# will-rowe/groot

Measured on AMD Instinct MI355X. Metric: Mreads/s aligned, higher is better.
Workload: dtype u64

## Files before the change

groot_amd/csrc/hip/ctx.hpp:

```cpp
#pragma once

#include <hip/hip_runtime.h>

#include <algorithm>
#include <array>
#include <atomic>
#include <cstdlib>
#include <deque>
#include <map>
#include <memory>
#include <string>
#include <thread>
#include <vector>

#include "device_types.hpp"

using namespace groot;


template <class T> struct DevBuf {
    T *p = nullptr;
    size_t n = 0;
    hipError_t alloc(size_t count)
    {
        release();
        n = count;
        return hipMalloc((void **)&p, std::max<size_t>(count, 1) * sizeof(T));
    }
    hipError_t reserve(size_t count) { return count <= n && p ? hipSuccess : alloc(count); }
    void swap(DevBuf &o) { std::swap(p, o.p); std::swap(n, o.n); }
// ... 15 lines not shown
        n = count;
        return hipHostMalloc((void **)&p, std::max<size_t>(count, 1) * sizeof(T), hipHostMallocDefault);
    }
    hipError_t reserve(size_t count) { return count <= n && p ? hipSuccess : alloc(count); }
    void release()
    {
        if (p) (void)hipHostFree(p);
        p = nullptr;
        n = 0;
    }
    ~PinBuf() { release(); }
};

struct Knobs {
    bool no_outcome_table = false, no_text_table = false, no_sig = false, force_rccl = false, small_buffers = false, open_stats = false, poison = false, lean = false, no_path = false,
         shared_slow = false, serial_tail = false, assign_global = false, library_sort = false;
    uint32_t ec_slots = 0;
    uint32_t acov_slots = 0;
    uint32_t rescue_ec_rows = 0;
    uint32_t rescue_acov_log = 0;
    static Knobs read()
    {
        Knobs k;
        k.no_outcome_table = getenv("GROOT_NO_OUTCOME_TABLE") != nullptr; k.no_text_table = getenv("GROOT_NO_TEXT_TABLE") != nullptr;
        k.no_sig = getenv("GROOT_NO_SIG") != nullptr;                     k.force_rccl = getenv("GROOT_FORCE_RCCL") != nullptr;
        k.small_buffers = getenv("GROOT_TEST_SMALL_BUFFERS") != nullptr;  k.open_stats = getenv("GROOT_OPEN_STATS") != nullptr;
        k.poison = getenv("GROOT_TEST_POISON") != nullptr;
        k.lean = getenv("GROOT_LEAN") != nullptr;
        k.no_path = getenv("GROOT_NO_PATH_PASS") != nullptr;
        k.shared_slow = getenv("GROOT_TEST_SHARED_SLOW") != nullptr;
        k.serial_tail = getenv("GROOT_SERIAL_TAIL") != nullptr;
        k.assign_global = getenv("GROOT_TEST_ASSIGN_GLOBAL") != nullptr;
        k.library_sort = getenv("GROOT_LIBRARY_SORT") != nullptr;
        if (const char *e = getenv("GROOT_TEST_EC_SLOTS")) k.ec_slots = (uint32_t)std::min<unsigned long>(strtoul(e, nullptr, 10), 1ul << 30);
        if (const char *e = getenv("GROOT_TEST_ACOV_SLOTS")) k.acov_slots = (uint32_t)std::min<unsigned long>(strtoul(e, nullptr, 10), 1ul << 30);
        if (const char *e = getenv("GROOT_TEST_RESCUE_EC_ROWS")) k.rescue_ec_rows = (uint32_t)std::min<unsigned long>(strtoul(e, nullptr, 10), 1ul << 30);
        if (const char *e = getenv("GROOT_TEST_RESCUE_ACOV_LOG")) k.rescue_acov_log = (uint32_t)std::min<unsigned long>(strtoul(e, nullptr, 10), 1ul << 28);
        return k;
    }
};

namespace groot {
struct EcTable;
struct AcovTable;
}

struct EcBufs {
    uint32_t cap = 0;
// ... 307 lines not shown
    uint32_t seed_slots = 0;
    DevBuf<uint32_t> sort_key, sort_key_out, perm_in, todo_list, todo_count;
    DevBuf<uint32_t> long_list, long_count;
    uint32_t vcap = 0;
    uint32_t lsh_defer_rows = 0, lsh_cap = 0;
    DevBuf<unsigned long long> seed_shards;
    DevBuf<uint32_t> lsh_list, lsh_count;
    DevBuf<uint64_t> lsh_sketch;
    DevBuf<char> sort_tmp, in_tmp;
    DevBuf<uint32_t> order_buf;
    size_t order_cap = 0;
    uint32_t order_dirty_n = 0, order_dirty_begin = 0, order_dirty_end = 0;
    uint32_t ovf_cap = 0;
    DevBuf<uint32_t> trav_off;
    DevBuf<char> scan_tmp;
    uint32_t align_threads = 0, stk_depth = 0;
    DevBuf<uint64_t> stk_hdr, stk_mask;
    DevBuf<uint32_t> attempts, q_row, q_seen, q_of_row, q_nrows;
    uint32_t *attempts_ptr = nullptr;
    uint32_t att_cap = 0;
    bool att_external = false;
    Counters ct;
};

#define HIP_TRY(ctx, expr)                                                                             \
    do {                                                                                                \
        hipError_t e__ = (expr);                                                                        \
        if (e__ != hipSuccess) return fail(ctx, GROOT_E_DEVICE, "%s: %s", #expr, hipGetErrorString(e__)); \
    } while (0)

// ... 18 lines not shown
```

groot_amd/csrc/hip/device_types.hpp:

```cpp
#pragma once

#include <cstdint>

#include <hip/hip_runtime.h>

#include "groot_hip.h"

namespace groot {

constexpr int kBlock = 256;
constexpr uint32_t kEmpty = 0xFFFFFFFFu;

enum : uint32_t {
    kFlagShortRead = 1u,
    kFlagLongRead = 2u,
    kFlagSeedOverflow = 4u,
    kFlagTravOverflow = 8u,
    kFlagOrdOverflow = 16u,
    kFlagOvfOverflow = 32u,
    kFlagQOverflow = 64u,
};

constexpr uint32_t kIncrCap = 8;
constexpr uint32_t kIncrCapBig = 2048;
constexpr uint32_t kSeedShards = 64, kSeedShardStride = 16;
constexpr uint32_t kOvfShards = 256;

struct DeviceCounters {
    unsigned long long mapped, multimapped, alignments, seeds, revcomp_panics, short_reads;
    unsigned int n_trav;
    unsigned int max_seeds;
    unsigned int flags;
    unsigned int q_rows;
    unsigned int mask_words;
    unsigned int todo_reads;
    unsigned int seeded_reads;
    unsigned int tab_reads;
    unsigned int lean_reads;
    unsigned int path_reads;
    unsigned int lsh_reads;
    unsigned int long_reads;
    unsigned long long dbg[192];
};

template <int PW> struct alignas(16) NodeRec {
    uint32_t seq_off;
    uint32_t seq_len;
    uint32_t deg;
    uint8_t child_first[4];
    uint64_t first8;
    uint32_t edges[4];
    uint64_t mask[PW];
};
static_assert(sizeof(NodeRec<3>) == 64, "node record must be one 64-byte line");
static_assert(sizeof(NodeRec<11>) == 128, "wide node record must be 128 bytes");

// ... 291 lines not shown
```

groot_amd/csrc/hip/groot_hip.hip:

```cpp
#include <cstring>

#include <hip/hip_runtime.h>
#include <rocprim/rocprim.hpp>

#include <dlfcn.h>

#include <algorithm>
#include <cmath>
#include <cstdarg>
#include <cstdio>
#include <atomic>
#include <chrono>
#include <deque>
#include <iterator>
#include <array>
#include <map>
#include <tuple>
#include <memory>
#include <numeric>
#include <string>
#include <thread>
#include <vector>

#include "../common/cpus.hpp"
// ... 272 lines not shown
        return GROOT_OK;
    }
    auto sort = [&](void *tmp) {
        return small_blocks ? rocprim::radix_sort_pairs<OrderSortConfig>(tmp, tmp_bytes, c->sort_key.p, c->sort_key_out.p, c->perm_in.p, w->perm.p, s->n_reads,
                                                                         begin_bit, end_bit, c->stream)
                            : rocprim::radix_sort_pairs(tmp, tmp_bytes, c->sort_key.p, c->sort_key_out.p, c->perm_in.p, w->perm.p, s->n_reads, begin_bit, end_bit,
                                                        c->stream);
    };
    HIP_TRY(c, sort(nullptr));
    if (tmp_bytes > c->sort_tmp.n) {
        HIP_TRY(c, hipStreamSynchronize(c->stream));
        HIP_TRY(c, c->sort_tmp.alloc(tmp_bytes + tmp_bytes / 4));
    }
    HIP_TRY(c, sort(c->sort_tmp.p));
    return GROOT_OK;
}

static int launch_align_stage(groot_ctx *c, Slot *s, bool update_weights)
{
    WorkSet *w = &c->ws[s->set];
    AlignArgs a{};
    a.ix = c->dix;
    a.seq = s->seq();
    a.seq_off = s->off();
    a.n_reads = s->n_reads;
    a.first_read_id = s->first_read_id;
    a.seed_slots = c->seed_slots;
    a.seed_count = w->seed_count.p;
    a.seed_win = w->seed_win.p;
    a.perm = w->perm.p;
// ... 6 lines not shown
    a.mask_first = w->mask_first.p;
    a.trav_cnt = w->trav_cnt.p;
    a.ovf_trav = w->ovf_trav.p;
    a.ovf_mask = w->ovf_mask.p;
    a.ovf_cnt = w->ovf_cnt.p;
    a.ovf_cap = c->ovf_cap;
    if (c->vcap) { a.vitem = w->vitem.p; a.vcount = w->vcount.p; a.vcap = c->vcap; }
    a.stk_hdr = c->stk_hdr.p;
    a.stk_mask = c->stk_mask.p;
    uint32_t blocks = std::min<uint32_t>((s->n_reads + kBlock - 1) / kBlock, c->align_threads / kBlock);
    if (c->dfs_frac < kSparseBelow && c->dfs_frac * (double)s->n_reads < 16.0 * (double)(blocks * (kBlock / 64))) blocks = std::max(1u, blocks / 2);
    else if (error_batch(c, s) && blocks >= 4) blocks /= 2;
    if ((s->lean_used || s->path_used) && c->lean_left_frac < 0.25) {
        uint32_t want = (uint32_t)(c->lean_left_frac * 1.25 * (double)s->n_reads / 64.0 / (kBlock / 64)) + 1u;
        blocks = std::max(1u, std::min(blocks, std::max(want, c->n_cu)));
    }
    a.n_threads = blocks * kBlock;
    a.stk_depth = c->stk_depth;
    {
        const uint32_t stride = (2 + 4 * ((s->max_len + 27) / 16)) | 1u;
        a.lds_stride_dw = (size_t)kBlock * stride * 4 <= 64 * 1024 ? stride : 0;
    }
    if (c->tab_capture) {
        a.incr_cnt = c->incr_cnt.p; a.incr_win = c->incr_win.p; a.incr_cap = c->incr_cap;
        HIP_TRY(c, hipMemsetAsync(c->incr_cnt.p, 0, (size_t)s->n_reads * sizeof(uint32_t), c->tstream));
    }
    a.head_lanes = s->mixed_len ? 16u : 0u;
#ifndef GROOT_REFILL_ERR
#define GROOT_REFILL_ERR 48
#endif
#ifndef GROOT_REFILL_MIXED
// ... 28 lines not shown
        a.perm = w->perm2.p;
        a.n_perm = l.left_cnt;
        a.rest = w->perm.p;
        a.rest_lo = lean_blocks * (uint32_t)kBlock;
        if (c->profiling) HIP_TRY(c, hipEventRecord(s->ev[13], c->astream));
        if (c->tstream != c->astream) {
            HIP_TRY(c, hipEventRecord(s->ev_walk, c->astream));
            HIP_TRY(c, hipStreamWaitEvent(c->tstream, s->ev_walk, 0));
        }
    }
    launch_align(c->pw, a, dim3(blocks), c->tstream);
    HIP_TRY(c, hipGetLastError());
    return GROOT_OK;
}

static int launch_order_stage(groot_ctx *c, Slot *s, bool update_weights)
{
    WorkSet *w = &c->ws[s->set];
    const uint32_t n = s->n_reads;
    size_t tmp_bytes = 0;
    if (c->vcap) hipLaunchKernelGGL(split_fix_kernel, dim3(256), dim3(kBlock), 0, c->tstream, w->split_list.p, w->vcount.p, w->vitem.p, w->trav_cnt.p, n, s->d_ctr.p,
                                    w->trav_first.p, w->mask_first.p, c->pw, s->first_read_id);
    HIP_TRY(c, rocprim::exclusive_scan(nullptr, tmp_bytes, w->trav_cnt.p, c->trav_off.p, 0u, n, rocprim::plus<uint32_t>(), c->tstream));
    if (tmp_bytes > c->scan_tmp.n) {
        HIP_TRY(c, hipStreamSynchronize(c->tstream));
        HIP_TRY(c, c->scan_tmp.alloc(tmp_bytes + tmp_bytes / 4));
    }
    HIP_TRY(c, rocprim::exclusive_scan(c->scan_tmp.p, tmp_bytes, w->trav_cnt.p, c->trav_off.p, 0u, n, rocprim::plus<uint32_t>(), c->tstream));
    OrderTabArgs ot{};
    if (c->dix.out_tab) {
        ot.tab_idx = w->tab_idx.p; ot.out_tab = c->dix.out_tab; ot.stride_q = c->dix.out_stride_q; ot.first_read_id = s->first_read_id;
        ot.update_weights = update_weights ? 1 : 0;
        ot.attempts = c->attempts_ptr; ot.q_row = c->q_row.p;
        ot.q_tab = c->dix.w - c->k + 1; ot.n_windows = c->n_windows;
    }
    if (c->profiling) HIP_TRY(c, hipEventRecord(s->ev[9], c->tstream));
    hipLaunchKernelGGL(order_first_kernel, dim3(std::min<uint32_t>((n + kBlock - 1) / kBlock, 2048u)), dim3(kBlock), 0, c->tstream, w->trav_first.p,
                       w->mask_first.p, c->trav_off.p, w->trav_cnt.p, n, s->d_trav.p, s->d_mask.p, s->trav_cap, c->pw,
                       c->pw_view, s->d_ctr.p, ot);
    if (c->profiling) HIP_TRY(c, hipEventRecord(s->ev[10], c->tstream));
    if (c->vcap) hipLaunchKernelGGL(order_split_kernel, dim3(std::min<uint32_t>((c->vcap + kBlock - 1) / kBlock, 256u)), dim3(kBlock), 0, c->tstream, w->vitem.p, w->vcount.p, c->vcap, w->trav_cnt.p,
                                    c->trav_off.p, w->trav_first.p, w->mask_first.p, n, s->first_read_id, s->d_trav.p, s->d_mask.p, s->trav_cap, c->pw, c->pw_view, s->d_ctr.p);
    hipLaunchKernelGGL(order_ovf_kernel, dim3((c->ovf_cap + kBlock - 1) / kBlock, kOvfShards), dim3(kBlock), 0, c->tstream,
                       w->ovf_trav.p, w->ovf_mask.p, w->ovf_cnt.p, c->ovf_cap, c->trav_off.p, s->first_read_id, s->d_trav.p,
                       s->d_mask.p, s->trav_cap, c->pw, c->pw_view, s->d_ctr.p, w->vitem.p, n, w->vcount.p);
    HIP_TRY(c, hipGetLastError());
    if (int rc = counters_assign(c, s)) return rc;
    if (!c->prm.results_on_device) {
        const dim3 g((s->trav_cap + kBlock - 1) / kBlock);
        hipLaunchKernelGGL(mask_words_kernel, g, dim3(kBlock), 0, c->tstream, s->d_trav.p, s->d_ctr.p, s->trav_cap, c->graph_words.p, (uint32_t)c->h_graph_words.size(),
                           s->d_mwords.p);
        size_t tb = 0;
        HIP_TRY(c, rocprim::exclusive_scan(nullptr, tb, s->d_mwords.p, s->d_moff.p, 0u, s->trav_cap, rocprim::plus<uint32_t>(), c->tstream));
        if (tb > c->scan_tmp.n) {
            HIP_TRY(c, hipStreamSynchronize(c->tstream));
            HIP_TRY(c, c->scan_tmp.alloc(tb + tb / 4));
        }
        HIP_TRY(c, rocprim::exclusive_scan(c->scan_tmp.p, tb, s->d_mwords.p, s->d_moff.p, 0u, s->trav_cap, rocprim::plus<uint32_t>(), c->tstream));
        hipLaunchKernelGGL(mask_compact_kernel, g, dim3(kBlock), 0, c->tstream, s->d_trav.p, s->d_mask.p, c->pw_view, s->d_ctr.p, s->trav_cap,
                           c->graph_words.p, (uint32_t)c->h_graph_words.size(), s->d_moff.p, s->d_cmask.p, s->d_ckpt.p);
// ... 284 lines not shown
        if (int rc = run_batch_async(c, s, redo_weights)) return rc;
        redone = true;
        DeviceCounters again{};
        if (int rc = refetch(again)) return rc;
        if (have_first) {
            const uint32_t keep = first.flags & ~(kFlagOvfOverflow | kFlagTravOverflow | kFlagSeedOverflow | kFlagQOverflow);
            DeviceCounters merged = first;
            merged.n_trav = again.n_trav; merged.alignments = again.alignments; merged.seeds = again.seeds; merged.max_seeds = again.max_seeds;
            merged.flags = keep | again.flags;
            merged.q_rows = again.q_rows;
            merged.mask_words = again.mask_words;
            merged.todo_reads = again.todo_reads; merged.tab_reads = again.tab_reads; merged.lean_reads = again.lean_reads; merged.path_reads = again.path_reads;
            h = merged;
        } else h = again;
    }
    s->n_trav = s->n_reads ? h.n_trav : 0;
    if (int rc = counters_collect(c, s, redone)) return rc;
    groot_counts &o = s->counts;
    o.received = s->n_reads;
    o.mapped = h.mapped; o.multimapped = h.multimapped; o.alignments = h.alignments; o.seeds = h.seeds;
    o.travs = s->n_trav; o.revcomp_panics = h.revcomp_panics; o.short_reads = h.short_reads;
    o.full_sketch_reads = (s->sig_used || s->text_used) ? h.todo_reads : s->n_reads;
    o.walked_reads = h.seeded_reads;
    o.lean_reads = h.lean_reads;
    s->path_reads = s->path_used ? h.path_reads : 0;
    if (s->status == GROOT_OK) {
        char buf[256];
        if (h.flags & kFlagLongRead) { s->status = GROOT_E_NOSPACE; snprintf(buf, sizeof buf, "a read is longer than max_read_len=%u", c->prm.max_read_len); s->status_msg = buf; }
        else if (h.flags & kFlagOrdOverflow) { s->status = GROOT_E_NOSPACE; s->status_msg = "a read produced more than 65535 traversals"; }
        else if (h.flags & kFlagShortRead) {
// ... 51 lines not shown
        fprintf(stderr, "[groot work] phase %d: %llu steps, %.2f us per step (wall clock, per wave)\n", ph, h.dbg[27 + ph],
                h.dbg[27 + ph] ? (double)h.dbg[24 + ph] / 100.0 / (double)h.dbg[27 + ph] : 0.0);
    for (int hh = 0; hh < 2; hh++) {
        fprintf(stderr, "[groot work] %s (buckets of 2 iterations):", hh ? "round length" : "lane finish");
        for (int b = 0; b < 64; b++) fprintf(stderr, " %llu", h.dbg[64 + 64 * hh + b]);
        fprintf(stderr, "\n");
    }
#endif
    if (s->n_reads) c->trav_per_read = (double)s->n_trav / (double)s->n_reads;
    if (s->n_reads && !c->tab_capture) c->dfs_frac = (double)h.seeded_reads / (double)s->n_reads;
    if (s->n_reads && !c->tab_capture && (s->lean_used || s->path_used)) {
        const uint32_t first = s->path_used ? h.path_reads : h.lean_reads;
        c->lean_left_frac = (double)(h.seeded_reads - std::min(h.seeded_reads, first)) / (double)s->n_reads;
    }
    if (s->n_reads && (s->sig_used || s->text_used)) c->todo_frac = (double)h.todo_reads / (double)s->n_reads;
    if (s->n_reads) { c->lsh_frac = (double)h.lsh_reads / (double)s->n_reads; c->long_frac = (double)h.long_reads / (double)s->n_reads; }
    if (s->n_reads && !c->tab_capture && c->dix.text_tab) {
        c->text_hit_frac = s->text_used ? 1.0 - (double)h.todo_reads / (double)s->n_reads : (double)h.tab_reads / (double)s->n_reads;
        if (s->text_used) c->text_retry_gap = c->text_hit_frac >= 0.7 ? 8u : std::min(256u, c->text_retry_gap * 2u);
    }
    s->n_mask_bytes = s->n_trav ? h.mask_words : 0;
    if (!c->prm.results_on_device && s->n_trav) {
        c->bytes_per_trav = (double)s->n_mask_bytes / (double)s->n_trav;
        const uint32_t have = redone ? 0 : std::min(s->copied, s->n_trav);
        if (have < s->n_trav) {
            if (c->packed_travs) HIP_TRY(c, hipMemcpy(s->h_ctrav.p + have, s->d_ctrav.p + have, (size_t)(s->n_trav - have) * sizeof(groot_ctrav), hipMemcpyDeviceToHost));
            else HIP_TRY(c, hipMemcpy(s->h_trav.p + have, s->d_trav.p + have, (size_t)(s->n_trav - have) * sizeof(groot_trav), hipMemcpyDeviceToHost));
            HIP_TRY(c, hipMemcpy(s->h_ckpt.p, s->d_ckpt.p, ((size_t)s->n_trav / 256 + 1) * sizeof(uint32_t), hipMemcpyDeviceToHost));
        }
        const uint64_t have_w = redone ? 0 : std::min<uint64_t>(s->copied_bytes, s->n_mask_bytes);
// ... 875 lines not shown
```

groot_amd/csrc/hip/kernels_cov.hpp:

```cpp
#pragma once

#include "kernels_common.hpp"

namespace groot {

struct CovArgs {
    const groot_trav *trav;
    const uint64_t *mask;
    const uint64_t *seq_off;
    const DeviceCounters *ctr;
    const uint32_t *node_np_off;
    const uint2 *np;
    const uint32_t *graph_path_off;
    const uint32_t *path_len;
    const uint64_t *slot_base;
    unsigned long long *starts, *ends;
    uint32_t cap, pw, first_read_id;
};

constexpr uint32_t kCovSkipFlags = kFlagSeedOverflow | kFlagTravOverflow | kFlagOvfOverflow | kFlagQOverflow | kFlagLongRead | kFlagOrdOverflow;

__global__ __launch_bounds__(kBlock) void cov_count_kernel(CovArgs a)
{
    if (a.ctr->flags & kCovSkipFlags) return;
    const uint32_t n = min(a.ctr->n_trav, a.cap);
    for (uint32_t t = blockIdx.x * kBlock + threadIdx.x; t < n; t += gridDim.x * kBlock) {
        const groot_trav tr = a.trav[t];
        const uint32_t r = tr.read_id - a.first_read_id;
        const uint64_t m = (a.seq_off[r + 1] - a.seq_off[r]) - ((tr.flags & GROOT_TRAV_START_CLIP) ? 1u : 0u) - ((tr.flags & GROOT_TRAV_END_CLIP) ? 1u : 0u);
        const uint32_t g0 = a.graph_path_off[tr.graph_id];
        const uint64_t *mk = a.mask + (size_t)t * a.pw;
        const uint32_t j1 = a.node_np_off[tr.node + 1];
        for (uint32_t j = a.node_np_off[tr.node]; j < j1; j++) {
            const uint2 e = a.np[j];
            if (!((mk[e.x >> 6] >> (e.x & 63)) & 1ull)) continue;
// ... 13 lines not shown
```

groot_amd/csrc/hip/kernels_misc.hpp:

```cpp
#pragma once

#include "kernels_common.hpp"

namespace groot {

__global__ __launch_bounds__(kBlock) void lsh_heavy_kernel(SeedArgs a)
{
    __shared__ uint64_t sk_lds[(kBlock / 64) * kLshHeavyMaxS];
    __shared__ uint32_t aux_lds[(kBlock / 64) * (2 * kLshMaxBands + 16)];
    const DeviceIndex &ix = a.ix;
    const uint32_t S = ix.s, maxk = ix.max_k, LB = ix.l_max, n = ix.n_windows;
    const uint32_t sl = S < kRowSlots ? S : kRowSlots, nd = (sl + 5) / 6;
    const uint32_t lane = threadIdx.x & 63, wave = threadIdx.x >> 6;
    uint64_t *m = sk_lds + wave * kLshHeavyMaxS;
    uint32_t *blo = aux_lds + wave * (2 * kLshMaxBands + 16);
    uint32_t *bcum = blo + kLshMaxBands;
    uint32_t *sc = bcum + kLshMaxBands + 1;
    auto wave_sync = []() { __builtin_amdgcn_fence(__ATOMIC_SEQ_CST, "wavefront"); __builtin_amdgcn_wave_barrier(); };
    const uint32_t n_list = min(*a.lsh_count, a.lsh_cap);
    for (uint32_t hi = blockIdx.x * (kBlock / 64) + wave; hi < n_list; hi += gridDim.x * (kBlock / 64)) {
        const uint32_t li = hi;
        const uint32_t e0 = a.lsh_list[li];
        const uint32_t r = e0 & 0x7FFFFFFFu, high = e0 >> 31;
        const uint64_t o0 = a.seq_off[r];
// ... 314 lines not shown

__global__ __launch_bounds__(kBlock) void fold_tab_hist_kernel(uint32_t *__restrict__ hist, uint32_t *__restrict__ attempts, const uint32_t *__restrict__ q_row,
                                                               uint32_t q_tab, uint32_t n_windows, const DeviceCounters *ctr, uint32_t update_weights)
{
    const bool live = update_weights && !(ctr->flags & (kFlagSeedOverflow | kFlagQOverflow));
    const uint32_t row = live ? q_row[q_tab] : kEmpty;
    for (uint32_t w = blockIdx.x * kBlock + threadIdx.x; w < n_windows; w += gridDim.x * kBlock) {
        const uint32_t v = hist[w];
        if (!v) continue;
        hist[w] = 0;
        if (row != kEmpty) atomicAdd(&attempts[(size_t)row * n_windows + w], v);
    }
}


struct OrderTabArgs {
    const uint32_t *tab_idx;
    const uint4 *out_tab;
    uint32_t stride_q, first_read_id;
    uint32_t update_weights;
    uint32_t *attempts;
    const uint32_t *q_row;
    uint32_t q_tab, n_windows;
};
__global__ __launch_bounds__(kBlock) void order_first_kernel(const groot_trav *first, const uint64_t *mask_first, const uint32_t *off,
                                                           const uint32_t *cnt, uint32_t n, groot_trav *out, uint64_t *mask_out,
                                                           uint32_t cap, uint32_t pw_in, uint32_t pw_out, DeviceCounters *ctr, OrderTabArgs t)
{
    __shared__ unsigned long long red[4];
    unsigned long long alns = 0, mapped = 0, multimapped = 0, seeds = 0;
    const bool live = !(ctr->flags & (kFlagSeedOverflow | kFlagQOverflow));
    if (blockIdx.x == 0 && threadIdx.x == 0 && n) ctr->n_trav = off[n - 1] + cnt[n - 1];
    for (uint32_t r = blockIdx.x * kBlock + threadIdx.x; r < n; r += gridDim.x * kBlock) {
    const uint32_t tw = t.tab_idx ? t.tab_idx[r] : kEmpty;
    const uint32_t ti = tw == kEmpty ? kEmpty : tw & ((1u << kOutIdxBits) - 1u);
    const bool count_here = (t.update_weights & 1u) && !(tw & kTabCounted);
    const bool seeds_here = tw != kEmpty && (tw & kTabSeedsHere);
    uint32_t ns = 0;
    if (ti != kEmpty && live) {
        const uint32_t nt = cnt[r], i = off[r];
        const bool fits = i < cap && nt <= cap - i;
        if (!fits) atomicOr(&ctr->flags, kFlagTravOverflow);
        const uint32_t row = t.update_weights ? t.q_row[t.q_tab] : 0u;
        uint32_t n_ent = nt ? nt : 1u;
        for (uint32_t j = 0; j < n_ent; j++) {
            const uint4 *e = t.out_tab + (size_t)(ti + j) * t.stride_q;
            uint4 h = e[0];
            if (j == 0) { n_ent += h.z >> 20; h.z &= 0xFFFFFu; }
            const uint4 x = e[1];
            const uint4 y = pw_out > 1 ? e[2] : make_uint4(0, 0, 0, 0);
            if (count_here) {
                if (x.x != kEmpty) atomicAdd(&t.attempts[(size_t)row * t.n_windows + x.x], 1u);
                if (x.y != kEmpty) atomicAdd(&t.attempts[(size_t)row * t.n_windows + x.y], 1u);
            }
            if (seeds_here) ns += (h.w >> 10) & 7u;
            if (j == 0) { mapped += (h.w >> 9) & 1u; multimapped += (h.w >> 8) & 1u; }
            if (j < nt) {
                alns += __popc(x.z) + __popc(x.w) + __popc(y.x) + __popc(y.y) + __popc(y.z) + __popc(y.w);
                if (pw_out > 3) {
                    const uint32_t *ew = reinterpret_cast<const uint32_t *>(e) + kOutHdrDw;
                    for (uint32_t w = 6; w < 2 * pw_out; w++) alns += __popc(ew[w]);
                }
            }
            if (!fits || j >= nt) continue;
            groot_trav tr;
            tr.read_id = t.first_read_id + r; tr.graph_id = h.z; tr.node = h.x; tr.offset = h.y;
            tr.ord = (uint16_t)j; tr.flags = (uint8_t)h.w; tr.reserved = 0;
            uint64_t *mo = mask_out + (size_t)(i + j) * pw_out;
            static_assert(sizeof(groot_trav) == 20, "record is five dwords");
            uint32_t tw5[5];
            __builtin_memcpy(tw5, &tr, 20);
            uint32_t *po = reinterpret_cast<uint32_t *>(out + i + j);
#pragma unroll
            for (int d = 0; d < 5; d++) __builtin_nontemporal_store(tw5[d], po + d);
            __builtin_nontemporal_store((uint64_t)x.z | ((uint64_t)x.w << 32), mo);
            if (pw_out > 1) __builtin_nontemporal_store((uint64_t)y.x | ((uint64_t)y.y << 32), mo + 1);
            if (pw_out > 2) __builtin_nontemporal_store((uint64_t)y.z | ((uint64_t)y.w << 32), mo + 2);
            const uint32_t *ew = reinterpret_cast<const uint32_t *>(e) + kOutHdrDw;
            for (uint32_t w = 3; w < pw_out; w++) mo[w] = (uint64_t)ew[2 * w] | ((uint64_t)ew[2 * w + 1] << 32);
        }
        if (seeds_here) seeds += ns;
    } else if (ti == kEmpty && cnt[r] != 0) {
        const uint32_t i = off[r];
        if (i >= cap) atomicOr(&ctr->flags, kFlagTravOverflow);
        else {
            out[i] = first[r];
            for (uint32_t w = 0; w < pw_out; w++) mask_out[(size_t)i * pw_out + w] = mask_first[(size_t)r * pw_in + w];
        }
    }
    }
    if (!t.tab_idx) return;
    alns = block_sum(alns, red);
    mapped = block_sum(mapped, red);
    multimapped = block_sum(multimapped, red);
    seeds = block_sum(seeds, red);
    if (threadIdx.x == 0) {
        if (alns) atomicAdd(&ctr->alignments, alns);
        if (seeds) atomicAdd(&ctr->seeds, seeds);
        if (t.update_weights) {
            if (mapped) atomicAdd(&ctr->mapped, mapped);
            if (multimapped) atomicAdd(&ctr->multimapped, multimapped);
        }
    }
}

__global__ __launch_bounds__(kBlock) void order_ovf_kernel(const groot_trav *ovf, const uint64_t *ovf_mask, const uint32_t *ovf_cnt,
                                                         uint32_t ovf_cap, const uint32_t *off, uint32_t first_read_id, groot_trav *out,
                                                         uint64_t *mask_out, uint32_t cap, uint32_t pw_in, uint32_t pw_out,
                                                         DeviceCounters *ctr, const uint4 *vitem, uint32_t n_reads, uint32_t *vcount)
{
    const uint32_t shard = blockIdx.y;
    const uint32_t slot = blockIdx.x * kBlock + threadIdx.x;
    if (!slot && !shard) { vcount[0] = 0; vcount[1] = 0; }
    if (slot >= min(ovf_cnt[shard], ovf_cap)) return;
    const size_t o = (size_t)shard * ovf_cap + slot;
    groot_trav t = ovf[o];
    uint32_t rid = t.read_id - first_read_id, ord = t.ord;
    if (rid >= n_reads) {
        const uint4 vi = vitem[rid - n_reads];
        rid = vi.x; ord += vi.w;
        t.read_id = first_read_id + rid;
        t.ord = (uint16_t)ord;
    }
    const uint32_t i = off[rid] + ord;
    if (i >= cap) { atomicOr(&ctr->flags, kFlagTravOverflow); return; }
    out[i] = t;
    for (uint32_t w = 0; w < pw_out; w++) mask_out[(size_t)i * pw_out + w] = ovf_mask[o * pw_in + w];
}

__global__ __launch_bounds__(kBlock) void mask_words_kernel(const groot_trav *__restrict__ trav, const DeviceCounters *ctr, uint32_t cap,
                                                          const uint8_t *__restrict__ graph_words, uint32_t n_graphs, uint32_t *__restrict__ words)
{
    const uint32_t i = blockIdx.x * kBlock + threadIdx.x;
    if (i >= cap) return;
    uint32_t w = 0;
    if (i < min(ctr->n_trav, cap)) {
        const uint32_t g = trav[i].graph_id;
        w = g < n_graphs ? graph_words[g] : 0u;
    }
    words[i] = w;
}
__global__ __launch_bounds__(kBlock) void mask_compact_kernel(const groot_trav *__restrict__ trav, const uint64_t *__restrict__ mask, uint32_t pw_in,
// ... 15 lines not shown
```

groot_amd/csrc/hip/open.hip:

```cpp
#include <hip/hip_runtime.h>

#include <algorithm>
#include <chrono>
#include <cstdio>
#include <cstring>
#include <memory>
#include <numeric>
#include <string>
#include <thread>
#include <vector>

#include "../common/cpus.hpp"
#include "../common/view_check.hpp"
#include "counters.hpp"
#include "ctx.hpp"
#include "index_tables.hpp"
#include "kernels_open.hpp"
#include "kernels_path.hpp"
#include "launch.hpp"
#include "open.hpp"

using namespace groot;

static int text_pass(groot_ctx *c, const uint8_t *seqs, const uint32_t *owner, uint32_t n, uint32_t len, uint8_t *differs, uint32_t *cnt_flags,
// ... 546 lines not shown
        HIP_TRY(c, w.perm_count.alloc(4));
        if (c->lean || c->path) {
            HIP_TRY(c, w.perm2.alloc(R));
            HIP_TRY(c, w.packed.alloc((size_t)R * (c->prm.max_read_len <= 128 ? 2 : 4)));
        }
        if (c->prm.keep_sketches) HIP_TRY(c, w.sketches.alloc((size_t)R * s));
        HIP_TRY(c, w.trav_first.alloc((size_t)R + c->vcap));
        HIP_TRY(c, w.mask_first.alloc(((size_t)R + c->vcap) * c->pw));
        HIP_TRY(c, w.trav_cnt.alloc((size_t)R + c->vcap));
        HIP_TRY(c, w.vitem.alloc(std::max<uint32_t>(c->vcap, 1)));
        HIP_TRY(c, w.split_list.alloc(kLongListCap));
        HIP_TRY(c, w.vcount.alloc(4));
        HIP_TRY(c, hipMemset(w.vcount.p, 0, 4 * sizeof(uint32_t)));
    }
    HIP_TRY(c, c->trav_off.alloc(R));
    if (c->lean || c->path) HIP_TRY(c, c->lean_stk.alloc((size_t)R * 4));
    if (c->path) HIP_TRY(c, c->path_hold.alloc((size_t)R * 3 * kPathHold));
    for (WorkSet &w : c->ws) {
        HIP_TRY(c, w.ovf_cnt.alloc(kOvfShards + 3));
        HIP_TRY(c, hipMemset(w.ovf_cnt.p, 0, (kOvfShards + 3) * sizeof(uint32_t)));
    }
    if (int rc = alloc_ovf(c, c->kn.small_buffers ? 2u : std::max<uint32_t>(256, R / kOvfShards / 4))) return rc;
    int n_cu = 256;
    (void)hipDeviceGetAttribute(&n_cu, hipDeviceAttributeMultiprocessorCount, c->device);
    c->n_cu = (uint32_t)std::max(n_cu, 1);
    uint32_t per_cu = c->pw > 3 ? kAlignWavesWide : kAlignWaves;
    c->align_threads = std::min<uint32_t>(((R + kBlock - 1) / kBlock) * kBlock, (uint32_t)std::max(n_cu, 1) * per_cu * kBlock);
    c->stk_depth = c->prm.max_read_len;
    HIP_TRY(c, c->stk_hdr.alloc((size_t)c->stk_depth * c->align_threads));
    HIP_TRY(c, c->stk_mask.alloc((size_t)c->stk_depth * c->align_threads * c->pw));
// ... 299 lines not shown
```

Baseline: 2449.

## Fuse exclusive scan into order placement kernel with decoupled look-back

```diff
diff --git a/groot_amd/csrc/hip/ctx.hpp b/groot_amd/csrc/hip/ctx.hpp
--- a/groot_amd/csrc/hip/ctx.hpp
+++ b/groot_amd/csrc/hip/ctx.hpp
@@ -14,6 +14,7 @@
 #include <vector>
 
 #include "device_types.hpp"
+#include "order_place_state.hpp"
 
 using namespace groot;
 
@@ -59,7 +60,9 @@
 
 struct Knobs {
     bool no_outcome_table = false, no_text_table = false, no_sig = false, force_rccl = false, small_buffers = false, open_stats = false, poison = false, lean = false, no_path = false,
-         shared_slow = false, serial_tail = false, assign_global = false, library_sort = false;
+         shared_slow = false, serial_tail = false, assign_global = false, library_sort = false, library_scan = false;
+    int tail_wg_per_cu = -1;
+    uint32_t tail_blocks = 0;
     uint32_t ec_slots = 0;
     uint32_t acov_slots = 0;
     uint32_t rescue_ec_rows = 0;
@@ -77,6 +80,9 @@
         k.serial_tail = getenv("GROOT_SERIAL_TAIL") != nullptr;
         k.assign_global = getenv("GROOT_TEST_ASSIGN_GLOBAL") != nullptr;
         k.library_sort = getenv("GROOT_LIBRARY_SORT") != nullptr;
+        k.library_scan = getenv("GROOT_LIBRARY_SCAN") != nullptr;
+        if (const char *e = getenv("GROOT_TAIL_WG_PER_CU")) k.tail_wg_per_cu = (int)std::min<unsigned long>(strtoul(e, nullptr, 10), 64ul);
+        if (const char *e = getenv("GROOT_TEST_TAIL_BLOCKS")) k.tail_blocks = (uint32_t)std::min<unsigned long>(strtoul(e, nullptr, 10), 1ul << 16);
         if (const char *e = getenv("GROOT_TEST_EC_SLOTS")) k.ec_slots = (uint32_t)std::min<unsigned long>(strtoul(e, nullptr, 10), 1ul << 30);
         if (const char *e = getenv("GROOT_TEST_ACOV_SLOTS")) k.acov_slots = (uint32_t)std::min<unsigned long>(strtoul(e, nullptr, 10), 1ul << 30);
         if (const char *e = getenv("GROOT_TEST_RESCUE_EC_ROWS")) k.rescue_ec_rows = (uint32_t)std::min<unsigned long>(strtoul(e, nullptr, 10), 1ul << 30);
@@ -414,6 +420,8 @@
     uint32_t ovf_cap = 0;
     DevBuf<uint32_t> trav_off;
     DevBuf<char> scan_tmp;
+    groot::order_place::State place;
+    int64_t ovf_longest = -1;
     uint32_t align_threads = 0, stk_depth = 0;
     DevBuf<uint64_t> stk_hdr, stk_mask;
     DevBuf<uint32_t> attempts, q_row, q_seen, q_of_row, q_nrows;
diff --git a/groot_amd/csrc/hip/device_types.hpp b/groot_amd/csrc/hip/device_types.hpp
--- a/groot_amd/csrc/hip/device_types.hpp
+++ b/groot_amd/csrc/hip/device_types.hpp
@@ -19,6 +19,7 @@
     kFlagOrdOverflow = 16u,
     kFlagOvfOverflow = 32u,
     kFlagQOverflow = 64u,
+    kFlagScanStall = 128u,
 };
 
 constexpr uint32_t kIncrCap = 8;
@@ -40,6 +41,7 @@
     unsigned int path_reads;
     unsigned int lsh_reads;
     unsigned int long_reads;
+    unsigned int ovf_longest;
     unsigned long long dbg[192];
 };
 
diff --git a/groot_amd/csrc/hip/groot_hip.hip b/groot_amd/csrc/hip/groot_hip.hip
--- a/groot_amd/csrc/hip/groot_hip.hip
+++ b/groot_amd/csrc/hip/groot_hip.hip
@@ -310,6 +310,11 @@
     }
     HIP_TRY(c, sort(c->sort_tmp.p));
     return GROOT_OK;
+}
+
+static uint32_t tail_wg_per_cu_default(const groot_ctx *, const Slot *)
+{
+    return 0;
 }
 
 static int launch_align_stage(groot_ctx *c, Slot *s, bool update_weights)
@@ -346,7 +351,10 @@
     if ((s->lean_used || s->path_used) && c->lean_left_frac < 0.25) {
         uint32_t want = (uint32_t)(c->lean_left_frac * 1.25 * (double)s->n_reads / 64.0 / (kBlock / 64)) + 1u;
         blocks = std::max(1u, std::min(blocks, std::max(want, c->n_cu)));
-    }
+        const uint32_t per_cu = c->kn.tail_wg_per_cu >= 0 ? (uint32_t)c->kn.tail_wg_per_cu : tail_wg_per_cu_default(c, s);
+        if (per_cu) blocks = std::max(1u, std::min(blocks, per_cu * c->n_cu));
+    }
+    if (c->kn.tail_blocks) blocks = std::max(1u, std::min(blocks, c->kn.tail_blocks));
     a.n_threads = blocks * kBlock;
     a.stk_depth = c->stk_depth;
     {
@@ -405,6 +413,14 @@
     return GROOT_OK;
 }
 
+static uint32_t ovf_blocks(uint32_t ovf_cap, int64_t longest)
+{
+    const uint32_t full = std::max<uint32_t>((ovf_cap + kBlock - 1) / kBlock, 1u);
+    if (longest < 0) return full;
+    const uint64_t want = ((uint64_t)longest + (uint64_t)longest / 4 + kBlock - 1) / kBlock;
+    return (uint32_t)std::min<uint64_t>(std::max<uint64_t>(want, 1), full);
+}
+
 static int launch_order_stage(groot_ctx *c, Slot *s, bool update_weights)
 {
     WorkSet *w = &c->ws[s->set];
@@ -412,12 +428,14 @@
     size_t tmp_bytes = 0;
     if (c->vcap) hipLaunchKernelGGL(split_fix_kernel, dim3(256), dim3(kBlock), 0, c->tstream, w->split_list.p, w->vcount.p, w->vitem.p, w->trav_cnt.p, n, s->d_ctr.p,
                                     w->trav_first.p, w->mask_first.p, c->pw, s->first_read_id);
-    HIP_TRY(c, rocprim::exclusive_scan(nullptr, tmp_bytes, w->trav_cnt.p, c->trav_off.p, 0u, n, rocprim::plus<uint32_t>(), c->tstream));
-    if (tmp_bytes > c->scan_tmp.n) {
-        HIP_TRY(c, hipStreamSynchronize(c->tstream));
-        HIP_TRY(c, c->scan_tmp.alloc(tmp_bytes + tmp_bytes / 4));
-    }
-    HIP_TRY(c, rocprim::exclusive_scan(c->scan_tmp.p, tmp_bytes, w->trav_cnt.p, c->trav_off.p, 0u, n, rocprim::plus<uint32_t>(), c->tstream));
+    if (c->kn.library_scan) {
+        HIP_TRY(c, rocprim::exclusive_scan(nullptr, tmp_bytes, w->trav_cnt.p, c->trav_off.p, 0u, n, rocprim::plus<uint32_t>(), c->tstream));
+        if (tmp_bytes > c->scan_tmp.n) {
+            HIP_TRY(c, hipStreamSynchronize(c->tstream));
+            HIP_TRY(c, c->scan_tmp.alloc(tmp_bytes + tmp_bytes / 4));
+        }
+        HIP_TRY(c, rocprim::exclusive_scan(c->scan_tmp.p, tmp_bytes, w->trav_cnt.p, c->trav_off.p, 0u, n, rocprim::plus<uint32_t>(), c->tstream));
+    }
     OrderTabArgs ot{};
     if (c->dix.out_tab) {
         ot.tab_idx = w->tab_idx.p; ot.out_tab = c->dix.out_tab; ot.stride_q = c->dix.out_stride_q; ot.first_read_id = s->first_read_id;
@@ -426,15 +444,14 @@
         ot.q_tab = c->dix.w - c->k + 1; ot.n_windows = c->n_windows;
     }
     if (c->profiling) HIP_TRY(c, hipEventRecord(s->ev[9], c->tstream));
-    hipLaunchKernelGGL(order_first_kernel, dim3(std::min<uint32_t>((n + kBlock - 1) / kBlock, 2048u)), dim3(kBlock), 0, c->tstream, w->trav_first.p,
-                       w->mask_first.p, c->trav_off.p, w->trav_cnt.p, n, s->d_trav.p, s->d_mask.p, s->trav_cap, c->pw,
-                       c->pw_view, s->d_ctr.p, ot);
+    HIP_TRY(c, order_place::launch(c->kn.library_scan ? nullptr : &c->place, w->trav_first.p, w->mask_first.p, c->trav_off.p, w->trav_cnt.p, n, s->d_trav.p, s->d_mask.p,
+                                   s->trav_cap, c->pw, c->pw_view, s->d_ctr.p, ot, c->tstream));
     if (c->profiling) HIP_TRY(c, hipEventRecord(s->ev[10], c->tstream));
     if (c->vcap) hipLaunchKernelGGL(order_split_kernel, dim3(std::min<uint32_t>((c->vcap + kBlock - 1) / kBlock, 256u)), dim3(kBlock), 0, c->tstream, w->vitem.p, w->vcount.p, c->vcap, w->trav_cnt.p,
                                     c->trav_off.p, w->trav_first.p, w->mask_first.p, n, s->first_read_id, s->d_trav.p, s->d_mask.p, s->trav_cap, c->pw, c->pw_view, s->d_ctr.p);
-    hipLaunchKernelGGL(order_ovf_kernel, dim3((c->ovf_cap + kBlock - 1) / kBlock, kOvfShards), dim3(kBlock), 0, c->tstream,
+    hipLaunchKernelGGL(order_ovf_kernel, dim3(ovf_blocks(c->ovf_cap, c->ovf_longest), kOvfShards), dim3(kBlock), 0, c->tstream,
                        w->ovf_trav.p, w->ovf_mask.p, w->ovf_cnt.p, c->ovf_cap, c->trav_off.p, s->first_read_id, s->d_trav.p,
-                       s->d_mask.p, s->trav_cap, c->pw, c->pw_view, s->d_ctr.p, w->vitem.p, n, w->vcount.p);
+                       s->d_mask.p, s->trav_cap, c->pw, c->pw_view, s->d_ctr.p, w->vitem.p, n, w->vcount.p, c->place.ticket);
     HIP_TRY(c, hipGetLastError());
     if (int rc = counters_assign(c, s)) return rc;
     if (!c->prm.results_on_device) {
@@ -749,6 +766,11 @@
             h = merged;
         } else h = again;
     }
+    if (s->n_reads && (h.flags & kFlagScanStall)) {
+        s->status = GROOT_E_DEVICE;
+        s->status_msg = "the order stage's look-back did not finish: the batch's records were not placed";
+        h.n_trav = 0;
+    }
     s->n_trav = s->n_reads ? h.n_trav : 0;
     if (int rc = counters_collect(c, s, redone)) return rc;
     groot_counts &o = s->counts;
@@ -830,6 +852,7 @@
         c->lean_left_frac = (double)(h.seeded_reads - std::min(h.seeded_reads, first)) / (double)s->n_reads;
     }
     if (s->n_reads && (s->sig_used || s->text_used)) c->todo_frac = (double)h.todo_reads / (double)s->n_reads;
+    if (s->n_reads) c->ovf_longest = h.ovf_longest;
     if (s->n_reads) { c->lsh_frac = (double)h.lsh_reads / (double)s->n_reads; c->long_frac = (double)h.long_reads / (double)s->n_reads; }
     if (s->n_reads && !c->tab_capture && c->dix.text_tab) {
         c->text_hit_frac = s->text_used ? 1.0 - (double)h.todo_reads / (double)s->n_reads : (double)h.tab_reads / (double)s->n_reads;
diff --git a/groot_amd/csrc/hip/kernels_cov.hpp b/groot_amd/csrc/hip/kernels_cov.hpp
--- a/groot_amd/csrc/hip/kernels_cov.hpp
+++ b/groot_amd/csrc/hip/kernels_cov.hpp
@@ -18,7 +18,7 @@
     uint32_t cap, pw, first_read_id;
 };
 
-constexpr uint32_t kCovSkipFlags = kFlagSeedOverflow | kFlagTravOverflow | kFlagOvfOverflow | kFlagQOverflow | kFlagLongRead | kFlagOrdOverflow;
+constexpr uint32_t kCovSkipFlags = kFlagSeedOverflow | kFlagTravOverflow | kFlagOvfOverflow | kFlagQOverflow | kFlagLongRead | kFlagOrdOverflow | kFlagScanStall;
 
 __global__ __launch_bounds__(kBlock) void cov_count_kernel(CovArgs a)
 {
diff --git a/groot_amd/csrc/hip/kernels_misc.hpp b/groot_amd/csrc/hip/kernels_misc.hpp
--- a/groot_amd/csrc/hip/kernels_misc.hpp
+++ b/groot_amd/csrc/hip/kernels_misc.hpp
@@ -1,6 +1,7 @@
 #pragma once
 
 #include "kernels_common.hpp"
+#include "order_place.hpp"
 
 namespace groot {
 
@@ -352,105 +353,18 @@
 }
 
 
-struct OrderTabArgs {
-    const uint32_t *tab_idx;
-    const uint4 *out_tab;
-    uint32_t stride_q, first_read_id;
-    uint32_t update_weights;
-    uint32_t *attempts;
-    const uint32_t *q_row;
-    uint32_t q_tab, n_windows;
-};
-__global__ __launch_bounds__(kBlock) void order_first_kernel(const groot_trav *first, const uint64_t *mask_first, const uint32_t *off,
-                                                           const uint32_t *cnt, uint32_t n, groot_trav *out, uint64_t *mask_out,
-                                                           uint32_t cap, uint32_t pw_in, uint32_t pw_out, DeviceCounters *ctr, OrderTabArgs t)
-{
-    __shared__ unsigned long long red[4];
-    unsigned long long alns = 0, mapped = 0, multimapped = 0, seeds = 0;
-    const bool live = !(ctr->flags & (kFlagSeedOverflow | kFlagQOverflow));
-    if (blockIdx.x == 0 && threadIdx.x == 0 && n) ctr->n_trav = off[n - 1] + cnt[n - 1];
-    for (uint32_t r = blockIdx.x * kBlock + threadIdx.x; r < n; r += gridDim.x * kBlock) {
-    const uint32_t tw = t.tab_idx ? t.tab_idx[r] : kEmpty;
-    const uint32_t ti = tw == kEmpty ? kEmpty : tw & ((1u << kOutIdxBits) - 1u);
-    const bool count_here = (t.update_weights & 1u) && !(tw & kTabCounted);
-    const bool seeds_here = tw != kEmpty && (tw & kTabSeedsHere);
-    uint32_t ns = 0;
-    if (ti != kEmpty && live) {
-        const uint32_t nt = cnt[r], i = off[r];
-        const bool fits = i < cap && nt <= cap - i;
-        if (!fits) atomicOr(&ctr->flags, kFlagTravOverflow);
-        const uint32_t row = t.update_weights ? t.q_row[t.q_tab] : 0u;
-        uint32_t n_ent = nt ? nt : 1u;
-        for (uint32_t j = 0; j < n_ent; j++) {
-            const uint4 *e = t.out_tab + (size_t)(ti + j) * t.stride_q;
-            uint4 h = e[0];
-            if (j == 0) { n_ent += h.z >> 20; h.z &= 0xFFFFFu; }
-            const uint4 x = e[1];
-            const uint4 y = pw_out > 1 ? e[2] : make_uint4(0, 0, 0, 0);
-            if (count_here) {
-                if (x.x != kEmpty) atomicAdd(&t.attempts[(size_t)row * t.n_windows + x.x], 1u);
-                if (x.y != kEmpty) atomicAdd(&t.attempts[(size_t)row * t.n_windows + x.y], 1u);
-            }
-            if (seeds_here) ns += (h.w >> 10) & 7u;
-            if (j == 0) { mapped += (h.w >> 9) & 1u; multimapped += (h.w >> 8) & 1u; }
-            if (j < nt) {
-                alns += __popc(x.z) + __popc(x.w) + __popc(y.x) + __popc(y.y) + __popc(y.z) + __popc(y.w);
-                if (pw_out > 3) {
-                    const uint32_t *ew = reinterpret_cast<const uint32_t *>(e) + kOutHdrDw;
-                    for (uint32_t w = 6; w < 2 * pw_out; w++) alns += __popc(ew[w]);
-                }
-            }
-            if (!fits || j >= nt) continue;
-            groot_trav tr;
-            tr.read_id = t.first_read_id + r; tr.graph_id = h.z; tr.node = h.x; tr.offset = h.y;
-            tr.ord = (uint16_t)j; tr.flags = (uint8_t)h.w; tr.reserved = 0;
-            uint64_t *mo = mask_out + (size_t)(i + j) * pw_out;
-            static_assert(sizeof(groot_trav) == 20, "record is five dwords");
-            uint32_t tw5[5];
-            __builtin_memcpy(tw5, &tr, 20);
-            uint32_t *po = reinterpret_cast<uint32_t *>(out + i + j);
-#pragma unroll
-            for (int d = 0; d < 5; d++) __builtin_nontemporal_store(tw5[d], po + d);
-            __builtin_nontemporal_store((uint64_t)x.z | ((uint64_t)x.w << 32), mo);
-            if (pw_out > 1) __builtin_nontemporal_store((uint64_t)y.x | ((uint64_t)y.y << 32), mo + 1);
-            if (pw_out > 2) __builtin_nontemporal_store((uint64_t)y.z | ((uint64_t)y.w << 32), mo + 2);
-            const uint32_t *ew = reinterpret_cast<const uint32_t *>(e) + kOutHdrDw;
-            for (uint32_t w = 3; w < pw_out; w++) mo[w] = (uint64_t)ew[2 * w] | ((uint64_t)ew[2 * w + 1] << 32);
-        }
-        if (seeds_here) seeds += ns;
-    } else if (ti == kEmpty && cnt[r] != 0) {
-        const uint32_t i = off[r];
-        if (i >= cap) atomicOr(&ctr->flags, kFlagTravOverflow);
-        else {
-            out[i] = first[r];
-            for (uint32_t w = 0; w < pw_out; w++) mask_out[(size_t)i * pw_out + w] = mask_first[(size_t)r * pw_in + w];
-        }
-    }
-    }
-    if (!t.tab_idx) return;
-    alns = block_sum(alns, red);
-    mapped = block_sum(mapped, red);
-    multimapped = block_sum(multimapped, red);
-    seeds = block_sum(seeds, red);
-    if (threadIdx.x == 0) {
-        if (alns) atomicAdd(&ctr->alignments, alns);
-        if (seeds) atomicAdd(&ctr->seeds, seeds);
-        if (t.update_weights) {
-            if (mapped) atomicAdd(&ctr->mapped, mapped);
-            if (multimapped) atomicAdd(&ctr->multimapped, multimapped);
-        }
-    }
-}
-
 __global__ __launch_bounds__(kBlock) void order_ovf_kernel(const groot_trav *ovf, const uint64_t *ovf_mask, const uint32_t *ovf_cnt,
                                                          uint32_t ovf_cap, const uint32_t *off, uint32_t first_read_id, groot_trav *out,
                                                          uint64_t *mask_out, uint32_t cap, uint32_t pw_in, uint32_t pw_out,
-                                                         DeviceCounters *ctr, const uint4 *vitem, uint32_t n_reads, uint32_t *vcount)
+                                                         DeviceCounters *ctr, const uint4 *vitem, uint32_t n_reads, uint32_t *vcount, uint32_t *place_ticket)
 {
     const uint32_t shard = blockIdx.y;
-    const uint32_t slot = blockIdx.x * kBlock + threadIdx.x;
-    if (!slot && !shard) { vcount[0] = 0; vcount[1] = 0; }
-    if (slot >= min(ovf_cnt[shard], ovf_cap)) return;
+    const uint32_t n_slots = min(ovf_cnt[shard], ovf_cap);
+    if (!blockIdx.x && !threadIdx.x) {
+        if (!shard) { vcount[0] = 0; vcount[1] = 0; if (place_ticket) *place_ticket = 0; }
+        if (n_slots) atomicMax(&ctr->ovf_longest, n_slots);
+    }
+    for (uint32_t slot = blockIdx.x * kBlock + threadIdx.x; slot < n_slots; slot += gridDim.x * kBlock) {
     const size_t o = (size_t)shard * ovf_cap + slot;
     groot_trav t = ovf[o];
     uint32_t rid = t.read_id - first_read_id, ord = t.ord;
@@ -461,9 +375,10 @@
         t.ord = (uint16_t)ord;
     }
     const uint32_t i = off[rid] + ord;
-    if (i >= cap) { atomicOr(&ctr->flags, kFlagTravOverflow); return; }
+    if (i >= cap) { atomicOr(&ctr->flags, kFlagTravOverflow); continue; }
     out[i] = t;
     for (uint32_t w = 0; w < pw_out; w++) mask_out[(size_t)i * pw_out + w] = ovf_mask[o * pw_in + w];
+    }
 }
 
 __global__ __launch_bounds__(kBlock) void mask_words_kernel(const groot_trav *__restrict__ trav, const DeviceCounters *ctr, uint32_t cap,
diff --git a/groot_amd/csrc/hip/open.hip b/groot_amd/csrc/hip/open.hip
--- a/groot_amd/csrc/hip/open.hip
+++ b/groot_amd/csrc/hip/open.hip
@@ -584,6 +584,7 @@
         HIP_TRY(c, hipMemset(w.vcount.p, 0, 4 * sizeof(uint32_t)));
     }
     HIP_TRY(c, c->trav_off.alloc(R));
+    HIP_TRY(c, order_place::reserve(c->place, R, nullptr));
     if (c->lean || c->path) HIP_TRY(c, c->lean_stk.alloc((size_t)R * 4));
     if (c->path) HIP_TRY(c, c->path_hold.alloc((size_t)R * 3 * kPathHold));
     for (WorkSet &w : c->ws) {
diff --git a/groot_amd/csrc/hip/order_place.hpp b/groot_amd/csrc/hip/order_place.hpp
--- /dev/null
+++ b/groot_amd/csrc/hip/order_place.hpp
@@ -0,0 +1,232 @@
+#pragma once
+
+#include <algorithm>
+
+#include "kernels_common.hpp"
+#include "order_place_state.hpp"
+
+namespace groot {
+
+struct OrderTabArgs {
+    const uint32_t *tab_idx;
+    const uint4 *out_tab;
+    uint32_t stride_q, first_read_id;
+    uint32_t update_weights;
+    uint32_t *attempts;
+    const uint32_t *q_row;
+    uint32_t q_tab, n_windows;
+};
+
+namespace order_place {
+
+constexpr uint32_t kAggregate = 1u, kInclusive = 2u;
+constexpr uint32_t kSpinMax = 1u << 22;
+
+struct PlaceScan {
+    unsigned long long *state;
+    uint32_t *ticket;
+    uint32_t epoch;
+};
+
+__host__ __device__ inline unsigned long long pack(uint32_t epoch, uint32_t st, uint32_t v)
+{
+    return ((unsigned long long)epoch << 34) | ((unsigned long long)st << 32) | v;
+}
+
+__device__ __forceinline__ uint32_t look_back(const PlaceScan &ps, uint32_t tile, uint32_t total, bool &ok)
+{
+    const uint32_t lane = threadIdx.x & 63;
+    if (lane == 0) __hip_atomic_store(&ps.state[tile], pack(ps.epoch, kAggregate, total), __ATOMIC_RELAXED, __HIP_MEMORY_SCOPE_AGENT);
+    uint32_t excl = 0;
+    ok = true;
+    for (int64_t hi = (int64_t)tile - 1; hi >= 0; hi -= 64) {
+        const int64_t idx = hi - lane;
+        unsigned long long w = 0, incl = 0, pending = 0;
+        uint32_t spins = 0;
+        for (;;) {
+            bool ready = true;
+            if (idx >= 0) {
+                w = __hip_atomic_load(&ps.state[idx], __ATOMIC_RELAXED, __HIP_MEMORY_SCOPE_AGENT);
+                ready = (uint32_t)(w >> 34) == ps.epoch && ((uint32_t)(w >> 32) & 3u) != 0;
+            }
+            incl = __ballot(idx >= 0 && ready && ((uint32_t)(w >> 32) & 3u) == kInclusive);
+            pending = __ballot(!ready);
+            if (!pending || (incl && __builtin_ctzll(incl) < __builtin_ctzll(pending))) break;
+            if (++spins > kSpinMax) { ok = false; break; }
+            __builtin_amdgcn_s_sleep(8);
+        }
+        const uint32_t stop = !ok ? (pending ? (uint32_t)__builtin_ctzll(pending) : 64u) : (incl ? (uint32_t)__builtin_ctzll(incl) + 1u : 64u);
+        uint32_t v = idx >= 0 && lane < stop ? (uint32_t)w : 0u;
+        for (int o = 32; o; o >>= 1) v += __shfl_xor(v, o);
+        excl += v;
+        if (!ok || incl) break;
+    }
+    if (lane == 0) __hip_atomic_store(&ps.state[tile], pack(ps.epoch, kInclusive, excl + total), __ATOMIC_RELAXED, __HIP_MEMORY_SCOPE_AGENT);
+    return excl;
+}
+
+}
+
+__global__ __launch_bounds__(kBlock, 8) void order_place_kernel(const groot_trav *first, const uint64_t *mask_first, uint32_t *off,
+                                                              const uint32_t *cnt, uint32_t n, groot_trav *out, uint64_t *mask_out,
+                                                              uint32_t cap, uint32_t pw_in, uint32_t pw_out, DeviceCounters *ctr, OrderTabArgs t,
+                                                              order_place::PlaceScan ps)
+{
+    using namespace order_place;
+    __shared__ unsigned long long red[4];
+    __shared__ uint32_t s_off[kTile + 1];
+    __shared__ uint32_t s_wave[kBlock / 64];
+    __shared__ uint32_t s_tile, s_excl;
+    unsigned long long alns = 0, mapped = 0, multimapped = 0, seeds = 0;
+    const bool live = !(ctr->flags & (kFlagSeedOverflow | kFlagQOverflow));
+    const uint32_t n_tiles = tiles(n), lane = threadIdx.x & 63, wave = threadIdx.x >> 6;
+    for (uint32_t it = 0;; it++) {
+    __syncthreads();
+    if (threadIdx.x == 0) s_tile = ps.state ? atomicAdd(ps.ticket, 1u) : blockIdx.x + it * gridDim.x;
+    __syncthreads();
+    const uint32_t tile = s_tile;
+    if (tile >= n_tiles) break;
+    const uint32_t base = tile * kTile, m = min(kTile, n - base);
+    if (!ps.state) {
+        for (uint32_t i = threadIdx.x; i < m; i += kBlock) s_off[i] = off[base + i];
+        if (threadIdx.x == 0) s_off[m] = base + m < n ? off[base + m] : off[n - 1] + cnt[n - 1];
+    } else {
+        const uint32_t i0 = threadIdx.x * kItems;
+        uint32_t v[kItems];
+        if (i0 + kItems <= m) {
+            const uint4 a = *reinterpret_cast<const uint4 *>(cnt + base + i0), b = *reinterpret_cast<const uint4 *>(cnt + base + i0 + 4);
+            v[0] = a.x; v[1] = a.y; v[2] = a.z; v[3] = a.w; v[4] = b.x; v[5] = b.y; v[6] = b.z; v[7] = b.w;
+        } else {
+#pragma unroll
+            for (uint32_t j = 0; j < kItems; j++) v[j] = i0 + j < m ? cnt[base + i0 + j] : 0u;
+        }
+        static_assert(kItems == 8, "two 16-byte loads per thread");
+        uint32_t mine = 0;
+#pragma unroll
+        for (uint32_t j = 0; j < kItems; j++) mine += v[j];
+        uint32_t incl = mine;
+        for (int o = 1; o < 64; o <<= 1) {
+            const uint32_t x = __shfl_up(incl, o);
+            if (lane >= (uint32_t)o) incl += x;
+        }
+        if (lane == 63) s_wave[wave] = incl;
+        __syncthreads();
+        uint32_t before = 0, total = 0;
+#pragma unroll
+        for (uint32_t k = 0; k < kBlock / 64; k++) { const uint32_t x = s_wave[k]; if (k < wave) before += x; total += x; }
+        if (wave == 0) {
+            uint32_t excl = 0;
+            if (tile == 0) {
+                if (lane == 0) __hip_atomic_store(&ps.state[0], pack(ps.epoch, kInclusive, total), __ATOMIC_RELAXED, __HIP_MEMORY_SCOPE_AGENT);
+            } else {
+                bool ok;
+                excl = look_back(ps, tile, total, ok);
+                if (!ok && lane == 0) atomicOr(&ctr->flags, kFlagScanStall);
+            }
+            if (lane == 0) s_excl = excl;
+        }
+        __syncthreads();
+        uint32_t o = s_excl + before + incl - mine;
+#pragma unroll
+        for (uint32_t j = 0; j < kItems; j++) {
+            if (i0 + j < m) s_off[i0 + j] = o;
+            o += v[j];
+        }
+        if (threadIdx.x == 0) s_off[m] = s_excl + total;
+    }
+    __syncthreads();
+    if (tile == n_tiles - 1 && threadIdx.x == 0) ctr->n_trav = s_off[m];
+#pragma nounroll
+    for (uint32_t li = threadIdx.x; li < m; li += kBlock) {
+    const uint32_t r = base + li, off_r = s_off[li], cnt_r = s_off[li + 1] - off_r;
+    if (ps.state) off[r] = off_r;
+    const uint32_t tw = t.tab_idx ? t.tab_idx[r] : kEmpty;
+    const uint32_t ti = tw == kEmpty ? kEmpty : tw & ((1u << kOutIdxBits) - 1u);
+    const bool count_here = (t.update_weights & 1u) && !(tw & kTabCounted);
+    const bool seeds_here = tw != kEmpty && (tw & kTabSeedsHere);
+    uint32_t ns = 0;
+    if (ti != kEmpty && live) {
+        const uint32_t nt = cnt_r, i = off_r;
+        const bool fits = i < cap && nt <= cap - i;
+        if (!fits) atomicOr(&ctr->flags, kFlagTravOverflow);
+        const uint32_t row = t.update_weights ? t.q_row[t.q_tab] : 0u;
+        uint32_t n_ent = nt ? nt : 1u;
+        for (uint32_t j = 0; j < n_ent; j++) {
+            const uint4 *e = t.out_tab + (size_t)(ti + j) * t.stride_q;
+            uint4 h = e[0];
+            if (j == 0) { n_ent += h.z >> 20; h.z &= 0xFFFFFu; }
+            const uint4 x = e[1];
+            const uint4 y = pw_out > 1 ? e[2] : make_uint4(0, 0, 0, 0);
+            if (count_here) {
+                if (x.x != kEmpty) atomicAdd(&t.attempts[(size_t)row * t.n_windows + x.x], 1u);
+                if (x.y != kEmpty) atomicAdd(&t.attempts[(size_t)row * t.n_windows + x.y], 1u);
+            }
+            if (seeds_here) ns += (h.w >> 10) & 7u;
+            if (j == 0) { mapped += (h.w >> 9) & 1u; multimapped += (h.w >> 8) & 1u; }
+            if (j < nt) {
+                alns += __popc(x.z) + __popc(x.w) + __popc(y.x) + __popc(y.y) + __popc(y.z) + __popc(y.w);
+                if (pw_out > 3) {
+                    const uint32_t *ew = reinterpret_cast<const uint32_t *>(e) + kOutHdrDw;
+                    for (uint32_t w = 6; w < 2 * pw_out; w++) alns += __popc(ew[w]);
+                }
+            }
+            if (!fits || j >= nt) continue;
+            groot_trav tr;
+            tr.read_id = t.first_read_id + r; tr.graph_id = h.z; tr.node = h.x; tr.offset = h.y;
+            tr.ord = (uint16_t)j; tr.flags = (uint8_t)h.w; tr.reserved = 0;
+            uint64_t *mo = mask_out + (size_t)(i + j) * pw_out;
+            static_assert(sizeof(groot_trav) == 20, "record is five dwords");
+            uint32_t tw5[5];
+            __builtin_memcpy(tw5, &tr, 20);
+            uint32_t *po = reinterpret_cast<uint32_t *>(out + i + j);
+#pragma unroll
+            for (int d = 0; d < 5; d++) __builtin_nontemporal_store(tw5[d], po + d);
+            __builtin_nontemporal_store((uint64_t)x.z | ((uint64_t)x.w << 32), mo);
+            if (pw_out > 1) __builtin_nontemporal_store((uint64_t)y.x | ((uint64_t)y.y << 32), mo + 1);
+            if (pw_out > 2) __builtin_nontemporal_store((uint64_t)y.z | ((uint64_t)y.w << 32), mo + 2);
+            const uint32_t *ew = reinterpret_cast<const uint32_t *>(e) + kOutHdrDw;
+            for (uint32_t w = 3; w < pw_out; w++) mo[w] = (uint64_t)ew[2 * w] | ((uint64_t)ew[2 * w + 1] << 32);
+        }
+        if (seeds_here) seeds += ns;
+    } else if (ti == kEmpty && cnt_r != 0) {
+        const uint32_t i = off_r;
+        if (i >= cap) atomicOr(&ctr->flags, kFlagTravOverflow);
+        else {
+            out[i] = first[r];
+            for (uint32_t w = 0; w < pw_out; w++) mask_out[(size_t)i * pw_out + w] = mask_first[(size_t)r * pw_in + w];
+        }
+    }
+    }
+    }
+    if (!t.tab_idx) return;
+    alns = block_sum(alns, red);
+    mapped = block_sum(mapped, red);
+    multimapped = block_sum(multimapped, red);
+    seeds = block_sum(seeds, red);
+    if (threadIdx.x == 0) {
+        if (alns) atomicAdd(&ctr->alignments, alns);
+        if (seeds) atomicAdd(&ctr->seeds, seeds);
+        if (t.update_weights) {
+            if (mapped) atomicAdd(&ctr->mapped, mapped);
+            if (multimapped) atomicAdd(&ctr->multimapped, multimapped);
+        }
+    }
+}
+
+namespace order_place {
+
+inline hipError_t launch(State *s, const groot_trav *first, const uint64_t *mask_first, uint32_t *off, const uint32_t *cnt, uint32_t n, groot_trav *out,
+                         uint64_t *mask_out, uint32_t cap, uint32_t pw_in, uint32_t pw_out, DeviceCounters *ctr, const OrderTabArgs &t, hipStream_t st)
+{
+    PlaceScan ps{};
+    if (s) {
+        if (tiles(n) > s->cap_tiles) return hipErrorInvalidValue;
+        ps.state = s->words; ps.ticket = s->ticket;
+        if (hipError_t e = next_epoch(*s, st, ps.epoch)) return e;
+    }
+    hipLaunchKernelGGL(order_place_kernel, dim3(grid(n)), dim3(kBlock), 0, st, first, mask_first, off, cnt, n, out, mask_out, cap, pw_in, pw_out, ctr, t, ps);
+    return hipGetLastError();
+}
+
+}
+}
diff --git a/groot_amd/csrc/hip/order_place_state.hpp b/groot_amd/csrc/hip/order_place_state.hpp
--- /dev/null
+++ b/groot_amd/csrc/hip/order_place_state.hpp
@@ -0,0 +1,59 @@
+#pragma once
+
+#include <hip/hip_runtime.h>
+
+#include <algorithm>
+#include <cstdint>
+
+namespace groot {
+namespace order_place {
+
+constexpr uint32_t kItems = 8;
+constexpr uint32_t kTile = kBlock * kItems;
+constexpr uint32_t kMaxBlocks = 2048;
+constexpr uint32_t kEpochBits = 30, kEpochMax = (1u << kEpochBits) - 1u;
+
+__host__ __device__ inline uint32_t tiles(uint32_t n) { return (n + kTile - 1) / kTile; }
+
+struct State {
+    unsigned long long *words = nullptr;
+    uint32_t *ticket = nullptr;
+    uint32_t cap_tiles = 0;
+    uint32_t epoch = 0;
+};
+
+inline size_t state_bytes(uint32_t cap_tiles) { return (size_t)cap_tiles * sizeof(unsigned long long) + 128; }
+
+inline void release(State &s)
+{
+    if (s.words) (void)hipFree(s.words);
+    s = State{};
+}
+
+inline hipError_t reserve(State &s, uint32_t n, hipStream_t st)
+{
+    const uint32_t want = std::max(tiles(n), 1u);
+    if (s.words && want <= s.cap_tiles) return hipSuccess;
+    release(s);
+    hipError_t e = hipMalloc((void **)&s.words, state_bytes(want));
+    if (e != hipSuccess) { s.words = nullptr; return e; }
+    s.cap_tiles = want;
+    s.ticket = reinterpret_cast<uint32_t *>(reinterpret_cast<char *>(s.words) + (size_t)want * sizeof(unsigned long long));
+    return hipMemsetAsync(s.words, 0, state_bytes(want), st);
+}
+
+inline hipError_t next_epoch(State &s, hipStream_t st, uint32_t &epoch)
+{
+    if (s.epoch >= kEpochMax) {
+        hipError_t e = hipMemsetAsync(s.words, 0, (size_t)s.cap_tiles * sizeof(unsigned long long), st);
+        if (e != hipSuccess) return e;
+        s.epoch = 0;
+    }
+    epoch = ++s.epoch;
+    return hipSuccess;
+}
+
+inline uint32_t grid(uint32_t n) { return std::max(1u, std::min(tiles(n), kMaxBlocks)); }
+
+}
+}
```

Result: no change. 2470 (median of 6 runs) (+0.9%).
